# tungphambasement/TNN

Measured on AMD Instinct MI355X. Metric: images/sec (whole node) WRN-16-8 on 32x32x3, pipeline-parallel, higher is better.
Workload: dtype bf16; 1 GPU; model=cifar100_wrn16_8, global_batch=256, input=32x32x3, microbatches=1, graphed_step=True, parallelism=single

## Files before the change

tnn_amd/csrc/bindings.cpp:

```cpp

#include <array>
#include <torch/extension.h>
#include <ATen/hip/HIPContext.h>

#include "kernels.h"

namespace tnn {

static hipStream_t cur_stream() {
  return at::hip::getCurrentHIPStreamMasqueradingAsCUDA().stream();
}

static void* zero_page(const at::Tensor& like) {
  static at::Tensor z;
  if (!z.defined() || z.device() != like.device())
    z = at::zeros({16}, like.options().dtype(at::kFloat));
  return z.data_ptr();
}

static DT dt_of(const at::Tensor& t) {
  if (t.scalar_type() == at::kFloat) return DT::F32;
  if (t.scalar_type() == at::kBFloat16) return DT::BF16;
  TORCH_CHECK(false, "tnn_amd kernels support fp32/bf16, got ", t.scalar_type());
}
// ... 424 lines not shown
                                         const at::Tensor& w,
                                         const c10::optional<at::Tensor>& bias,
                                         int64_t sh, int64_t sw, int64_t ph,
                                         int64_t pw) {
  return conv2d_fwd_impl(x, w, bias, sh, sw, ph, pw, false, true);
}

at::Tensor conv2d_dgrad(const at::Tensor& dy, const at::Tensor& w, int64_t H,
                        int64_t W, int64_t sh, int64_t sw, int64_t ph,
                        int64_t pw) {
  CHECK_IN(dy);
  CHECK_IN(w);
  int KH = w.size(0), KW = w.size(1), Cin = w.size(2), Cout = w.size(3);
  auto cs = conv_shape_out(dy.size(0), H, W, Cin, Cout, KH, KW, sh, sw, ph, pw,
                           dy.size(1), dy.size(2));
  auto dx = at::empty({cs.N, H, W, Cin}, dy.options());
  if (conv2d_dgrad_wants_db(dt_of(dy), dy.data_ptr(), cs)) {
    auto w_t2d = at::empty({Cin, (int64_t)KH * KW * Cout}, w.options());
    transpose_w_dgrad_launch(dt_of(w), w.data_ptr(), w_t2d.data_ptr(), KH * KW,
                             Cin, Cout, cur_stream());
    conv2d_dgrad_launch(dt_of(dy), dy.data_ptr(), nullptr, w_t2d.data_ptr(),
                        dx.data_ptr(), zero_page(dy), cs, cur_stream());
    return dx;
  }
  auto w_t = at::empty({KH, KW, Cout, Cin}, w.options());
  transpose_w_launch(dt_of(w), w.data_ptr(), w_t.data_ptr(), KH, KW, Cin, Cout,
                     cur_stream());
  conv2d_dgrad_launch(dt_of(dy), dy.data_ptr(), w_t.data_ptr(), nullptr,
                      dx.data_ptr(), zero_page(dy), cs, cur_stream());
  return dx;
}

std::string conv2d_fwd_route_name(const at::Tensor& x, const at::Tensor& w,
                                  int64_t sh, int64_t sw, int64_t ph,
                                  int64_t pw, bool stats) {
  CHECK_IN(x);
  CHECK_IN(w);
  auto cs = conv_shape(x, w.size(2), w.size(3), w.size(0), w.size(1), sh, sw,
                       ph, pw);
  return conv2d_fwd_route(dt_of(x), x.data_ptr(), cs, stats);
}

std::string conv2d_dgrad_route_name(const at::Tensor& dy,
                                    const at::Tensor& w, int64_t H, int64_t W,
                                    int64_t sh, int64_t sw, int64_t ph,
                                    int64_t pw) {
  CHECK_IN(dy);
  CHECK_IN(w);
  auto cs = conv_shape_out(dy.size(0), H, W, w.size(2), w.size(3), w.size(0),
                           w.size(1), sh, sw, ph, pw, dy.size(1), dy.size(2));
  return conv2d_dgrad_route(dt_of(dy), dy.data_ptr(), cs);
}

static at::Tensor conv2d_wgrad_rows(const at::Tensor& x, const at::Tensor& dy,
                                    int64_t KH, int64_t KW, int64_t sh,
                                    int64_t sw, int64_t ph, int64_t pw,
                                    bool out_in_dt, bool bias) {
  CHECK_IN(x);
  CHECK_IN(dy);
  auto cs = conv_shape(x, x.size(3), dy.size(3), KH, KW, sh, sw, ph, pw);
  TORCH_CHECK(dy.size(1) == cs.OH && dy.size(2) == cs.OW, "wgrad shape");
  DT out_dt = out_in_dt ? dt_of(x) : DT::F32;
  const int64_t rows = KH * KW * cs.Cin + (bias ? 1 : 0);
  auto out = at::empty({rows, (int64_t)cs.Cout},
                       out_dt == DT::F32 ? x.options().dtype(at::kFloat)
                                         : x.options());
  int z = conv2d_wgrad_zsplits(cs);
  at::Tensor ws;
  float* wsp = nullptr;
  if (z > 1 || out_dt != DT::F32) {
    ws = at::empty({(int64_t)z * rows * cs.Cout},
                   x.options().dtype(at::kFloat));
    wsp = ws.data_ptr<float>();
  }
  conv2d_wgrad_launch(dt_of(x), x.data_ptr(), dy.data_ptr(), out.data_ptr(),
                      out_dt, wsp, z, zero_page(x), cs, bias, cur_stream());
  return out;
}

at::Tensor conv2d_wgrad(const at::Tensor& x, const at::Tensor& dy, int64_t KH,
                        int64_t KW, int64_t sh, int64_t sw, int64_t ph,
                        int64_t pw, bool out_in_dt) {
  return conv2d_wgrad_rows(x, dy, KH, KW, sh, sw, ph, pw, out_in_dt, false)
      .view({KH, KW, x.size(3), dy.size(3)});
}

std::vector<at::Tensor> conv2d_wgrad_bias(const at::Tensor& x,
                                          const at::Tensor& dy, int64_t KH,
                                          int64_t KW, int64_t sh, int64_t sw,
                                          int64_t ph, int64_t pw,
                                          bool out_in_dt) {
  auto out = conv2d_wgrad_rows(x, dy, KH, KW, sh, sw, ph, pw, out_in_dt, true);
  const int64_t kout = out.size(0) - 1;
  return {out.narrow(0, 0, kout).view({KH, KW, x.size(3), dy.size(3)}),
          out.select(0, kout)};
}

std::vector<at::Tensor> bn_fwd_train(const at::Tensor& x,
                                     const at::Tensor& gamma,
                                     const at::Tensor& beta,
                                     const c10::optional<at::Tensor>& rmean,
                                     const c10::optional<at::Tensor>& rvar,
                                     double momentum, double eps, bool relu,
                                     double dropout_p, int64_t seed,
                                     const c10::optional<at::Tensor>& precomp,
                                     const c10::optional<at::Tensor>& ctr =
                                         c10::nullopt) {
  CHECK_IN(x);
  TORCH_CHECK(dropout_p == 0.0 || relu, "fused BN dropout requires relu");
  int C = x.size(-1);
  int64_t rows = x.numel() / C;
  auto mean = at::empty({C}, x.options().dtype(at::kFloat));
  auto invstd = at::empty({C}, x.options().dtype(at::kFloat));
  auto y = at::empty_like(x);
  float* rm = rmean.has_value() ? rmean->data_ptr<float>() : nullptr;
  float* rv = rvar.has_value() ? rvar->data_ptr<float>() : nullptr;
  if (precomp.has_value()) {
    TORCH_CHECK(precomp->numel() == 2 * C, "bad precomputed stats");
    const float* ps = precomp->data_ptr<float>();
    bn_finalize_launch(ps, ps + C, mean.data_ptr<float>(),
// ... 778 lines not shown
  TORCH_CHECK(step.is_cuda() && step.scalar_type() == at::kLong &&
              step.numel() == 1, "sample_logits step must be int64 [1]");
  const float* up = nullptr;
  if (u.has_value()) {
    TORCH_CHECK(u->is_cuda() && u->is_contiguous() &&
                u->scalar_type() == at::kFloat && u->numel() == R,
                "sample_logits u must be fp32 [R] on device");
    up = u->data_ptr<float>();
  }
  auto ids = at::empty({R}, logits.options().dtype(at::kLong));
  if (R > 0)
    sample_logits_launch(logits.data_ptr(), ids.data_ptr<int64_t>(), (int)R,
                         (int)V, (float)temperature,
                         (int)std::min<int64_t>(top_k, V), (float)top_p,
                         (uint64_t)seed, step.data_ptr<int64_t>(), up,
                         cur_stream());
  return ids;
}

namespace imgcodec {
at::Tensor decode_image(const py::bytes& data);
}

}

PYBIND11_MODULE(TORCH_EXTENSION_NAME, m) {
  m.def("act_fwd", &tnn::act_fwd);
  m.def("act_bwd", &tnn::act_bwd);
  m.def("relu_bwd_mask", &tnn::relu_bwd_mask);
  m.def("add_act_fwd", &tnn::add_act_fwd);
  m.def("add_act_bwd", &tnn::add_act_bwd);
  m.def("dropout_fwd", &tnn::dropout_fwd, py::arg("x"), py::arg("p"),
        py::arg("seed"), py::arg("ctr") = c10::nullopt);
  m.def("dropout_bwd", &tnn::dropout_bwd);
  m.def("colsum", &tnn::colsum);
  m.def("gemm", &tnn::gemm, py::arg("a"), py::arg("b"), py::arg("bias"),
        py::arg("act_kind"), py::arg("residual") = c10::nullopt,
        py::arg("ln_gamma") = c10::nullopt, py::arg("ln_beta") = c10::nullopt,
        py::arg("ln_eps") = 1e-5);
  m.def("gemm_skinny", &tnn::gemm_skinny, py::arg("a"), py::arg("b"),
        py::arg("bias"), py::arg("act_kind"),
        py::arg("residual") = c10::nullopt, py::arg("ln_gamma") = c10::nullopt,
        py::arg("ln_beta") = c10::nullopt, py::arg("ln_eps") = 1e-5);
  m.def("skinny_enabled", &tnn::skinny_enabled);
  m.def("gemm_nt", &tnn::gemm_nt);
  m.def("gemm_tn", &tnn::gemm_tn);
  m.def("mfma_selftest", &tnn::mfma_selftest);
  m.def("mfma_selftest_f32", &tnn::mfma_selftest_f32);
  m.def("conv2d_fwd", &tnn::conv2d_fwd);
  m.def("conv2d_fwd_stats", &tnn::conv2d_fwd_stats);
  m.def("conv2d_dgrad", &tnn::conv2d_dgrad);
  m.def("conv2d_fwd_route", &tnn::conv2d_fwd_route_name);
  m.def("conv2d_dgrad_route", &tnn::conv2d_dgrad_route_name);
  m.def("conv2d_wgrad", &tnn::conv2d_wgrad);
  m.def("conv2d_wgrad_bias", &tnn::conv2d_wgrad_bias);
  m.def("bn_fwd_train", &tnn::bn_fwd_train, py::arg("x"), py::arg("gamma"),
        py::arg("beta"), py::arg("rmean"), py::arg("rvar"),
        py::arg("momentum"), py::arg("eps"), py::arg("relu"),
        py::arg("dropout_p"), py::arg("seed"), py::arg("precomp"),
        py::arg("ctr") = c10::nullopt);
  m.def("bn_fwd_infer", &tnn::bn_fwd_infer);
  m.def("bn_bwd", &tnn::bn_bwd, py::arg("x"), py::arg("dy"),
        py::arg("gamma"), py::arg("mean"), py::arg("invstd"),
        py::arg("y_relu"), py::arg("dy_scale"),
        py::arg("resid") = py::none());
  m.def("maxpool_fwd", &tnn::maxpool_fwd);
  m.def("maxpool_bwd", &tnn::maxpool_bwd);
  m.def("avgpool_fwd", &tnn::avgpool_fwd);
  m.def("avgpool_bwd", &tnn::avgpool_bwd);
  m.def("ce_fwd", &tnn::ce_fwd);
  m.def("ce_bwd", &tnn::ce_bwd);
  m.def("ptloss_fwd", &tnn::ptloss_fwd);
  m.def("ptloss_bwd", &tnn::ptloss_bwd);
  m.def("gn_fwd", &tnn::gn_fwd);
  m.def("gn_bwd", &tnn::gn_bwd);
  m.def("ln_fwd", &tnn::ln_fwd);
  m.def("ln_bwd", &tnn::ln_bwd, py::arg("x"), py::arg("dy"),
        py::arg("gamma"), py::arg("mean"), py::arg("invstd"),
        py::arg("resid") = py::none());
  m.def("embedding_fwd", &tnn::embedding_fwd);
  m.def("embedding_bwd", &tnn::embedding_bwd);
  m.def("attn_fwd", &tnn::attn_fwd);
  m.def("attn_bwd", &tnn::attn_bwd, py::arg("q"), py::arg("k"),
        py::arg("v"), py::arg("o"), py::arg("dout"), py::arg("lse"),
        py::arg("causal"), py::arg("dq_out") = py::none(),
        py::arg("dk_out") = py::none(), py::arg("dv_out") = py::none());
  m.def("bmm", &tnn::bmm);
  m.def("smax_fwd", &tnn::smax_fwd);
  m.def("smax_bwd", &tnn::smax_bwd);
  m.def("attn_decode", &tnn::attn_decode);
  m.def("kv_append", &tnn::kv_append);
  m.def("attn_extend", &tnn::attn_extend);
  m.def("kv_append_n", &tnn::kv_append_n);
  m.def("sample_logits", &tnn::sample_logits, py::arg("logits"),
        py::arg("temperature"), py::arg("top_k"), py::arg("top_p"),
        py::arg("seed"), py::arg("step"), py::arg("u") = c10::nullopt);
  m.def("sgd_step", &tnn::sgd_step, py::arg("param"), py::arg("master"),
        py::arg("grad"), py::arg("momentum_buf"), py::arg("lr"),
        py::arg("momentum"), py::arg("weight_decay"), py::arg("nesterov"),
        py::arg("clip") = c10::nullopt, py::arg("lr_dev") = c10::nullopt);
  m.def("adam_step", &tnn::adam_step, py::arg("param"), py::arg("master"),
        py::arg("grad"), py::arg("m"), py::arg("v"), py::arg("step"),
        py::arg("lr"), py::arg("beta1"), py::arg("beta2"), py::arg("eps"),
        py::arg("weight_decay"), py::arg("adamw"),
        py::arg("step_dev") = c10::nullopt, py::arg("clip") = c10::nullopt,
        py::arg("lr_dev") = c10::nullopt);
// ... 16 lines not shown
```

tnn_amd/csrc/conv2d.hip:

```cpp

#include "common.h"
#include "kernels.h"
#include "tile_gemm.h"

namespace tnn {

using namespace tile;

template <bool POW2>
DEV int idiv(int x, const IDiv& f) {
  if constexpr (POW2) return x >> f.lg;
  else if (f.magic)
    return (int)(((unsigned long long)(unsigned)x * f.magic) >> f.sh);
  else
    return x / f.d;
}
template <bool POW2>
DEV int imod(int x, const IDiv& f) {
  if constexpr (POW2) return x & (f.d - 1);
  else return x - idiv<POW2>(x, f) * f.d;
}

DEV void kdecode(int kidx, const ConvShape& cs, int& kh, int& kw) {
  kh = (kidx * cs.mkw16) >> 16;
// ... 167 lines not shown
  });
}

template <typename T, typename S>
DEV void conv_fwd_stats(const WaveCoordT<S>& wc, f32x4 acc[S::FM][S::FN],
                        const T* bias_p, float* stats, const ConvShape& cs,
                        int m0, int n0, int M) {
  constexpr int FM = S::FM, FN = S::FN;
  float* ssum = stats;
  float* ssumsq = stats + cs.Cout;
  const int cr = (wc.lane >> 4) * 4;
  const int cc = wc.lane & 15;
#pragma unroll
  for (int fn = 0; fn < FN; ++fn) {
    int col = n0 + wc.wcol0 + fn * 16 + cc;
    float bias = 0.0f;
    if (col < cs.Cout) {
      if (bias_p) bias = VecIO<T>::to_f32(bias_p[col]);
    }
    float s = 0.0f, ss = 0.0f;
#pragma unroll
    for (int fm = 0; fm < FM; ++fm)
#pragma unroll
      for (int j = 0; j < 4; ++j) {
        int row = m0 + wc.wrow0 + fm * 16 + cr + j;
        if (row < M && col < cs.Cout) {
          float v = acc[fm][fn][j] + bias;
          s += v;
          ss += v * v;
        }
      }
    s += __shfl_xor(s, 16, 64);
    ss += __shfl_xor(ss, 16, 64);
    s += __shfl_xor(s, 32, 64);
    ss += __shfl_xor(ss, 32, 64);
    if (wc.lane < 16 && col < cs.Cout) {
      atomicAdd(&ssum[col], s);
      atomicAdd(&ssumsq[col], ss);
    }
  }
}

template <bool POW2, typename T, bool S2, typename S>
DEV void dgrad_store(const WaveCoordT<S>& wc, f32x4 acc[S::FM][S::FN], T* DX,
                     const ConvShape& cs, const DgradClass<S2>& dc, int m0,
                     int n0) {
  epilogue_visit(wc, acc, m0, n0, [&](int row, int col, float v) {
    if (row < dc.M && col < cs.Cin)
      DX[dc.template pixel<POW2>(cs, row) * cs.Cin + col] =
          VecIO<T>::from_f32(v);
  });
}

DEV float* wgrad_slab_store(const WaveCoord& wc, f32x4 acc[FM][FN],
                            float* DW, const ConvShape& cs, int Kout,
                            int bias_row, int r0, int n0) {
  float* out = DW + (int64_t)blockIdx.z * (Kout + bias_row) * cs.Cout;
  epilogue_visit(wc, acc, r0, n0, [&](int row, int col, float v) {
    if (row < Kout && col < cs.Cout) out[(int64_t)row * cs.Cout + col] = v;
  });
  return out;
}
DEV void wgrad_colsum_store(float* out, const ConvShape& cs, int Kout, int n0,
                            float bsum) {
  bsum = colsum_tile_finish(bsum);
  int col = n0 + (threadIdx.x >> 2);
  if ((threadIdx.x & 3) == 0 && col < cs.Cout)
    out[(int64_t)Kout * cs.Cout + col] = bsum;
}

template <bool DB, typename T, typename S, typename RowFn, typename TapFn,
          typename AtFn>
DEV void conv_db_kloop(T* As0, T* As1, T* Bs0, T* Bs1,
                       const WaveCoordT<S>& wc, f32x4 acc[S::FM][S::FN],
                       const T* __restrict__ asrc, int lgSW, int lgC,
                       const T* __restrict__ bsrc, int64_t bstride,
                       int brows, int m0, int n0, int K,
                       const T* __restrict__ zero16, RowFn&& row,
                       TapFn&& tap, AtFn&& at) {
  constexpr int NA = glds_count<T, S::BM>();
  constexpr int NB = glds_count<T, S::BN>();
  constexpr int NPER = NA + NB;
  const int wid = __builtin_amdgcn_readfirstlane(wc.wid);
  const bool uni = lgC >= 6;

  const T* ab[NA];
  int ap[NA], aq[NA];
  const T* bb[NB];
  bool bok[NB];
#pragma unroll
  for (int i = 0; i < NA; ++i) {
    const int j = wid * NA + i;
    int64_t noff;
    int p, q;
    const bool ok = row(m0 + glds_row<T>(j, wc.lane), noff, p, q);
    ab[i] = asrc + noff + (uni ? glds_kk<T>(j, wc.lane) : 0);
    ap[i] = ok ? p : -(1 << 28);
    aq[i] = q;
  }
#pragma unroll
  for (int i = 0; i < NB; ++i) {
    const int j = wid * NB + i;
    const int gn = n0 + glds_row<T>(j, wc.lane);
    bok[i] = gn < brows;
    bb[i] = bsrc + (int64_t)gn * bstride + (uni ? glds_kk<T>(j, wc.lane) : 0);
  }

  auto a_ptr = [&](int i, int dh, int dw, int c, bool& ok) {
    int sh, sw;
    ok = at(ap[i], aq[i], dh, dw, sh, sw);
    const unsigned pix = ((unsigned)sh << lgSW) + (unsigned)sw;
    return ab[i] + (int)((pix << lgC) + (unsigned)c);
  };
  auto stage = [&](int t, T* a_img, T* b_img) {
// ... 451 lines not shown
      int c = threadIdx.x + it * THREADS;
      int mm = c / (BM / V);
      int rr = (c % (BM / V)) * V;
      int gm = k0 + mm, gr = r0 + rr;
      asrc[it] = gm < m_end && gr < Kout
                     ? fwd_src<true>(X, cs, fwd_row<true>(cs, gm), gr, zero16)
                     : zero16;
    }
    const T* bsrc[RB];
#pragma unroll
    for (int it = 0; it < RB; ++it) {
      int c = threadIdx.x + it * THREADS;
      int mm = c / (BN / V);
      int nn = (c % (BN / V)) * V;
      int gm = k0 + mm;
      bsrc[it] = (gm < m_end && n0 + nn + V <= cs.Cout)
                     ? &DY[(int64_t)gm * cs.Cout + n0 + nn]
                     : zero16;
    }
#pragma unroll
    for (int it = 0; it < RA; ++it) va[it] = *(const VecT*)asrc[it];
#pragma unroll
    for (int it = 0; it < RB; ++it) vb[it] = *(const VecT*)bsrc[it];
  };

  load_tile(m_begin);
  for (int k0 = m_begin; k0 < m_end; k0 += BK) {
#pragma unroll
    for (int it = 0; it < RA; ++it) {
      int c = threadIdx.x + it * THREADS;
      int mm = c / (BM / V);
      int rr = (c % (BM / V)) * V;
#pragma unroll
      for (int j = 0; j < V; ++j) As[lds_off<T>(rr + j, mm)] = va[it].e[j];
    }
#pragma unroll
    for (int it = 0; it < RB; ++it) {
      int c = threadIdx.x + it * THREADS;
      int mm = c / (BN / V);
      int nn = (c % (BN / V)) * V;
#pragma unroll
      for (int j = 0; j < V; ++j) Bs[lds_off<T>(nn + j, mm)] = vb[it].e[j];
    }
    if (k0 + BK < m_end) load_tile(k0 + BK);
    __syncthreads();
    mfma_compute_tile(As, Bs, wc, acc);
    if (colsum) bsum += colsum_tile_partial(Bs);
    __syncthreads();
  }
  float* out = wgrad_slab_store(wc, acc, DW, cs, Kout, bias_row, r0, n0);
  if (colsum) wgrad_colsum_store(out, cs, Kout, n0, bsum);
}

__launch_bounds__(THREADS, 2)
__global__ void k_conv_wgrad_tr(const bf16* __restrict__ X,
                                const bf16* __restrict__ DY,
                                float* __restrict__ DW,
                                const bf16* __restrict__ zero16, ConvShape cs,
                                int bias_row) {
  constexpr int NA = glds_kmajor_count<BM / 8>();
  constexpr int NPER = NA + glds_kmajor_count<BN / 8>();
  __shared__ alignas(16) bf16 As0[BK * BM], As1[BK * BM];
  __shared__ alignas(16) bf16 Bs0[BK * BN], Bs1[BK * BN];
  const int M = cs.N * cs.OH * cs.OW;
  const int Kout = cs.KH * cs.KW * cs.Cin;
  int tr_, tn_;
  conv_tile_order(cs, tr_, tn_);
  const int r0 = tr_ * BM;
  const int n0 = tn_ * BN;
  const int m_begin = (int)((int64_t)M * blockIdx.z / gridDim.z);
  const int m_end = (int)((int64_t)M * (blockIdx.z + 1) / gridDim.z);
  const WaveCoord wc;
  const int wm = wc.wid / WAVES_N;
  f32x4 acc[FM][FN] = {};
  const bool colsum = bias_row && tr_ == 0;
  f32x4 bacc = {};
  bf16x8 ones;
#pragma unroll
  for (int j = 0; j < 8; ++j) ones[j] = (__bf16)1.0f;

  int a_dh[NA], a_dw[NA], a_ci[NA];
#pragma unroll
  for (int i = 0; i < NA; ++i) {
    const int row = 4 * (wc.wid * NA + i) + wc.lane / 16;
    const int gr = r0 + 8 * ((wc.lane % 16) ^ kmaj_key<16>(row));
    int kh, kw;
    kdecode(gr >> cs.d_cin.lg, cs, kh, kw);
    a_dh[i] = kh - cs.PH;
    a_dw[i] = kw - cs.PW;
    a_ci[i] = gr < Kout ? (gr & (cs.Cin - 1)) : -1;
  }

  auto stage = [&](int k0, bf16* a_img, bf16* b_img) {
    glds_stage_kmajor<BM / 8>(a_img, wc,
                              [&](int i, int row, int) -> const bf16* {
      const int gm = k0 + row;
      const int n = gm >> cs.d_ohow.lg;
      const int rem = gm & (cs.OH * cs.OW - 1);
      const int oh = rem >> cs.d_ow.lg, ow = rem & (cs.OW - 1);
      const int ih = oh * cs.SH + a_dh[i];
      const int iw = ow * cs.SW + a_dw[i];
      const bool ok = gm < m_end && a_ci[i] >= 0 &&
                      (unsigned)ih < (unsigned)cs.H &&
                      (unsigned)iw < (unsigned)cs.W;
      const int pix = (n << cs.d_hw.lg) + (ih << cs.d_w.lg) + iw;
      const bf16* p = X + (((int64_t)pix << cs.d_cin.lg) + a_ci[i]);
      return ok ? p : zero16;
    });
    glds_stage_kmajor<BN / 8>(b_img, wc,
                              [&](int, int row, int ch) -> const bf16* {
      const int gm = k0 + row, gn = n0 + 8 * ch;
      const bf16* p = DY + (((int64_t)gm << cs.d_cout.lg) + gn);
      return gm < m_end && gn < cs.Cout ? p : zero16;
    });
  };
  auto compute = [&](const bf16* a_img, const bf16* b_img) {
#pragma unroll
    for (int ks = 0; ks < BK / 32; ++ks) {
      TrFrag a[FM], b[FN];
#pragma unroll
      for (int fm = 0; fm < FM; ++fm)
        a[fm] = tr_frag_issue<BM / 8>(a_img, ks * 32, wc.wrow0 + fm * 16,
                                      wc.lane);
#pragma unroll
      for (int fn = 0; fn < FN; ++fn)
        b[fn] = tr_frag_issue<BN / 8>(b_img, ks * 32, wc.wcol0 + fn * 16,
                                      wc.lane);
      tr_frags_wait(a, b);
#pragma unroll
      for (int fm = 0; fm < FM; ++fm)
#pragma unroll
        for (int fn = 0; fn < FN; ++fn)
          acc[fm][fn] = __builtin_amdgcn_mfma_f32_16x16x32_bf16(
              a[fm].get(), b[fn].get(), acc[fm][fn], 0, 0, 0);
      if (colsum)
        bacc = __builtin_amdgcn_mfma_f32_16x16x32_bf16(
            ones, wm ? b[1].get() : b[0].get(), bacc, 0, 0, 0);
    }
  };

  auto step = [&](int k0, bf16* a_cur, bf16* b_cur, bf16* a_nxt,
                  bf16* b_nxt) {
    if (k0 + BK < m_end) {
      stage(k0 + BK, a_nxt, b_nxt);
      wait_vmcnt<NPER>();
    } else {
      wait_vmcnt<0>();
    }
    __builtin_amdgcn_s_barrier();
    compute(a_cur, b_cur);
    __builtin_amdgcn_s_barrier();
  };
  if (m_begin < m_end) stage(m_begin, As0, Bs0);
  for (int k0 = m_begin; k0 < m_end; k0 += 2 * BK) {
    step(k0, As0, Bs0, As1, Bs1);
    if (k0 + BK < m_end) step(k0 + BK, As1, Bs1, As0, Bs0);
  }

  float* out = wgrad_slab_store(wc, acc, DW, cs, Kout, bias_row, r0, n0);
  if (colsum && wc.lane < 16) {
    int col = n0 + wc.wcol0 + 16 * wm + wc.lane;
    if (col < cs.Cout) out[(int64_t)Kout * cs.Cout + col] = bacc[0];
  }
}

template <typename T>
__global__ void k_transpose2d_tiled(const T* __restrict__ in,
                                    T* __restrict__ out, int rows, int cols) {
  __shared__ T tile[32][33];
  const int c0 = blockIdx.x * 32, r0 = blockIdx.y * 32;
  const int64_t slice = (int64_t)blockIdx.z * rows * cols;
  const T* src = in + slice;
  T* dst = out + slice;
  const int tx = threadIdx.x & 31, ty = threadIdx.x >> 5;
#pragma unroll
  for (int d = 0; d < 32; d += 8) {
    int r = r0 + ty + d, c = c0 + tx;
    if (r < rows && c < cols) tile[ty + d][tx] = src[(int64_t)r * cols + c];
  }
  __syncthreads();
#pragma unroll
  for (int d = 0; d < 32; d += 8) {
    int c = c0 + ty + d, r = r0 + tx;
    if (c < cols && r < rows) dst[(int64_t)c * rows + r] = tile[tx][ty + d];
  }
}

template <typename T>
__global__ void k_transpose_w_dgrad(const T* __restrict__ W,
                                    T* __restrict__ WT2D, int KHW, int Cin,
                                    int Cout) {
  int64_t i = (int64_t)blockIdx.x * blockDim.x + threadIdx.x;
  int64_t n = (int64_t)KHW * Cin * Cout;
  if (i >= n) return;
  int co = i % Cout;
  int ci = (i / Cout) % Cin;
  int64_t khw = i / ((int64_t)Cin * Cout);
  WT2D[((int64_t)ci * KHW + khw) * Cout + co] = W[i];
}

template <typename T>
__global__ void k_transpose_w_dgrad_vec(const T* __restrict__ W,
                                        T* __restrict__ WT2D, int KHW,
                                        int Cin, int Cout) {
  constexpr int V = 16 / sizeof(T);
  struct alignas(16) P { T e[16 / sizeof(T)]; };
  const int cov = Cout / V;
  int64_t i = (int64_t)blockIdx.x * blockDim.x + threadIdx.x;
  int64_t n = (int64_t)KHW * Cin * cov;
  if (i >= n) return;
  int c = i % cov;
  int ci = (i / cov) % Cin;
  int64_t khw = i / ((int64_t)Cin * cov);
  ((P*)WT2D)[((int64_t)ci * KHW + khw) * cov + c] =
      ((const P*)W)[((int64_t)khw * Cin + ci) * cov + c];
// ... 223 lines not shown
  dim3 grid(ceil_div(M, BM), ceil_div(cs.Cin, BN));
  bool p2 = all_pow2(cs);
  bool g = p2 && vec_ok(dt, dy, cs.Cout);
  bool s1 = cs.SH == 1 && cs.SW == 1;
  ConvShape cs2;
  bool s2 = dgrad_parity(cs, cs2);
  int Mc = cs.N * (cs.H / 2) * (cs.W / 2);
  dim3 grid_s2(ceil_div(Mc, BM), ceil_div(cs.Cin, BN), 4);
  const Wide wide = dgrad_wide(dt, w_t2d != nullptr, s2, cs);
  dispatch_dt(dt, [&](auto tag) {
    using T = typename decltype(tag)::type;
    auto DY = (const T*)dy;
    auto DX = (T*)dx;
    auto Z = (const T*)zero16;
    if constexpr (sizeof(T) == 2) {
      if (wide != Wide::NO) {
        auto WT = (const T*)w_t2d;
        constexpr int WBM = TileWide::BM, WBN = TileWide::BN;
        const bool sb = wide == Wide::SB;
        if (s2)
          return launch(sb ? k_conv_dgrad_sb_wide<true>
                           : k_conv_dgrad_db_wide<true>,
                        dim3(ceil_div(Mc, WBM), cs.Cin / WBN, 4), s, DY, WT,
                        DX, Z, cs2);
        dim3 gw(ceil_div(M, WBM), cs.Cin / WBN);
        if (s1)
          return launch(sb ? k_conv_dgrad_sb_wide<false, true>
                           : k_conv_dgrad_db_wide<false, true>,
                        gw, s, DY, WT, DX, Z, cs);
        return launch(sb ? k_conv_dgrad_sb_wide<> : k_conv_dgrad_db_wide<>,
                      gw, s, DY, WT, DX, Z, cs);
      }
    }
    if (w_t2d) {
      auto WT = (const T*)w_t2d;
      if (s2)
        return launch(k_conv_dgrad_db<T, true>, grid_s2, s, DY, WT, DX, Z,
                      cs2);
      return launch(s1 ? k_conv_dgrad_db<T, false, true> : k_conv_dgrad_db<T>,
                    grid, s, DY, WT, DX, Z, cs);
    }
    auto WT = (const T*)w_t;
    if (g && s2)
      return launch(k_conv_dgrad<T, true, true, true>, grid_s2, s, DY, WT, DX,
                    Z, cs2);
    launch(g ? (s1 ? k_conv_dgrad<T, true, true, false, true>
                   : k_conv_dgrad<T, true, true>)
             : (p2 ? k_conv_dgrad<T, true, false>
                   : k_conv_dgrad<T, false, false>),
           grid, s, DY, WT, DX, Z, cs);
  });
}

int conv2d_wgrad_zsplits(const ConvShape& cs) {
  int M = cs.N * cs.OH * cs.OW;
  int Kout = cs.KH * cs.KW * cs.Cin;
  int base = ceil_div(Kout, BM) * ceil_div(cs.Cout, BN);
  int want = 2048;
  int z = base >= want ? 1
                       : std::min(ceil_div(M, 4 * BK), ceil_div(want, base));
  return std::max(z, 1);
}

void conv2d_wgrad_launch(DT dt, const void* x, const void* dy, void* dw_out,
                         DT out_dt, float* ws, int z, const void* zero16,
                         const ConvShape& cs, bool bias, hipStream_t s) {
  int Kout = cs.KH * cs.KW * cs.Cin;
  const int bias_row = bias ? 1 : 0;
  bool direct = z == 1 && out_dt == DT::F32;
  float* target = direct ? (float*)dw_out : ws;
  dim3 grid(ceil_div(Kout, BM), ceil_div(cs.Cout, BN), z);
  bool p2 = all_pow2(cs);
  bool vec = p2 && vec_ok(dt, x, cs.Cin) && vec_ok(dt, dy, cs.Cout);
  dispatch_dt(dt, [&](auto tag) {
    using T = typename decltype(tag)::type;
    auto X = (const T*)x;
    auto DY = (const T*)dy;
    auto Z = (const T*)zero16;
    if (vec) {
      if constexpr (sizeof(T) == 2)
        launch(k_conv_wgrad_tr, grid, s, X, DY, target, Z, cs, bias_row);
      else
        launch(k_conv_wgrad_vec<T>, grid, s, X, DY, target, Z, cs, bias_row);
      return;
    }
    launch(p2 ? k_conv_wgrad<T, true> : k_conv_wgrad<T, false>, grid, s, X,
           DY, target, cs, bias_row);
  });
  if (!direct)
    splitk_reduce_launch(ws, dw_out, out_dt, z,
                         (int64_t)(Kout + bias_row) * cs.Cout, s,
                         (int64_t)Kout * cs.Cout);
}

}
```

tnn_amd/csrc/kernels.h:

```cpp
#pragma once

#include <hip/hip_runtime.h>
#ifdef __HIPCC__
#include <hip/hip_bf16.h>
#endif
#include <algorithm>
#include <cstdint>

namespace tnn {

enum class DT { F32, BF16 };

inline bool ptr_aligned16(const void* p) { return ((uintptr_t)p & 15) == 0; }

inline int vec_elems(DT dt) { return dt == DT::F32 ? 4 : 8; }

#ifdef __HIPCC__
template <typename T> struct TypeTag { using type = T; };
template <typename F>
inline void dispatch_dt(DT dt, F&& f) {
  if (dt == DT::F32) f(TypeTag<float>{});
  else f(TypeTag<__hip_bfloat16>{});
}
#endif
// ... 62 lines not shown
                          int64_t n, hipStream_t s, int64_t n_shape = 0);
void mfma_selftest_launch(const void* a_bf16, const void* b_bf16, float* d,
                          hipStream_t s);
void mfma_selftest_f32_launch(const float* a, const float* b, float* d,
                              hipStream_t s);

struct IDiv {
  int d = 1;
  int lg = 0;
  int sh = 0;
  unsigned long long magic = 0;
  void set(int dd) {
    d = dd;
    lg = (dd & (dd - 1)) == 0 ? __builtin_ctz(dd) : -1;
    magic = 0;
    sh = 0;
    if (lg < 0 && dd > 1 && dd < 65536) {
      sh = dd < 1024 ? 36 : 42;
      magic = ((1ull << sh) + dd - 1) / dd;
    }
  }
};

struct ConvShape {
  int N, H, W, Cin, Cout, KH, KW, SH, SW, PH, PW, OH, OW;
  IDiv d_ohow, d_ow, d_cin, d_hw, d_w, d_cout;
  int mkw16;
  void init_fdiv() {
    d_ohow.set(OH * OW);
    d_ow.set(OW);
    d_cin.set(Cin);
    d_hw.set(H * W);
    d_w.set(W);
    d_cout.set(Cout);
    mkw16 = 65536 / KW + 1;
  }
};
bool conv2d_fwd_wants_db(DT dt, const void* x, const ConvShape& cs);
void transpose_w_fwd_launch(DT dt, const void* w, void* w_t2, int KHW, int Cin,
                            int Cout, hipStream_t s);
void conv2d_fwd_launch(DT dt, const void* x, const void* w, const void* w_t2,
                       const void* bias, void* y, const void* zero16,
                       float* stats, const ConvShape& cs, bool relu,
                       hipStream_t s);
bool conv2d_dgrad_wants_db(DT dt, const void* dy, const ConvShape& cs);
const char* conv2d_fwd_route(DT dt, const void* x, const ConvShape& cs,
                             bool stats);
const char* conv2d_dgrad_route(DT dt, const void* dy, const ConvShape& cs);
void transpose_w_dgrad_launch(DT dt, const void* w, void* w_t2d, int KHW,
                              int Cin, int Cout, hipStream_t s);
void conv2d_dgrad_launch(DT dt, const void* dy, const void* w_t,
                         const void* w_t2d, void* dx, const void* zero16,
                         const ConvShape& cs, hipStream_t s);
int conv2d_wgrad_zsplits(const ConvShape& cs);
void conv2d_wgrad_launch(DT dt, const void* x, const void* dy, void* dw_out,
                         DT out_dt, float* ws, int z, const void* zero16,
                         const ConvShape& cs, bool bias, hipStream_t s);
void transpose_w_launch(DT dt, const void* w, void* w_t, int KH, int KW,
                        int Cin, int Cout, hipStream_t s);

int64_t bn_stats_ws_floats(DT dt, const void* x, int64_t rows, int cols);
void bn_stats_launch(DT dt, const void* x, float* mean, float* invstd,
                     float* rmean, float* rvar, float momentum, float* ws,
                     int64_t rows, int cols, float eps, hipStream_t s);
void bn_finalize_launch(const float* sum, const float* sumsq, float* mean,
                        float* invstd, float* rmean, float* rvar,
                        float momentum, int64_t rows, int cols, float eps,
                        hipStream_t s);
void bn_apply_launch(DT dt, const void* x, const float* mean,
                     const float* invstd, const float* gamma, const float* beta,
                     void* y, int64_t rows, int cols, bool relu, hipStream_t s);
void bn_apply_drop_launch(DT dt, const void* x, const float* mean,
                          const float* invstd, const float* gamma,
                          const float* beta, void* y, int64_t rows, int cols,
                          float p, uint64_t seed, const int64_t* ctr,
                          hipStream_t s);
void bn_infer_launch(DT dt, const void* x, const float* rmean,
                     const float* rvar, const float* gamma, const float* beta,
                     void* y, int64_t rows, int cols, float eps, bool relu,
                     hipStream_t s);
int64_t bn_bwd_ws_floats(DT dt, const void* x, const void* dy, int64_t rows,
                         int cols);
void bn_bwd_reduce_launch(DT dt, const void* x, const void* dy, const void* y_relu,
                          const float* mean, const float* invstd, float* sum_dy,
                          float* sum_dy_xhat, float* ws, int64_t rows, int cols,
                          float dy_scale, hipStream_t s);
void bn_bwd_apply_launch(DT dt, const void* x, const void* dy, const void* y_relu,
                         const float* mean, const float* invstd,
                         const float* gamma, const float* sum_dy,
                         const float* sum_dy_xhat, void* dx, const void* resid,
                         int64_t rows, int cols, float dy_scale,
                         hipStream_t s);

struct PoolShape {
  int N, H, W, C, KH, KW, SH, SW, PH, PW, OH, OW;
};
void maxpool_fwd_launch(DT dt, const void* x, void* y, int32_t* idx,
                        const PoolShape& ps, hipStream_t s);
void maxpool_bwd_launch(DT dt, const void* dy, const int32_t* idx, float* dx_f32,
                        const PoolShape& ps, hipStream_t s);
void avgpool_fwd_launch(DT dt, const void* x, void* y, const PoolShape& ps,
                        hipStream_t s);
void avgpool_bwd_launch(DT dt, const void* dy, void* dx, const PoolShape& ps,
                        hipStream_t s);

void ce_fwd_launch(DT dt, const void* logits, const int64_t* targets,
                   float* loss, float* lse, int64_t rows, int cols,
// ... 109 lines not shown
```

tnn_amd/csrc/tile_gemm.h:

```cpp
#pragma once

#include "common.h"

namespace tile {

constexpr int BK = 64, THREADS = 256;

template <int BM_, int BN_, int WAVES_M_ = 2, int WAVES_N_ = 2>
struct TileShape {
  static constexpr int BM = BM_, BN = BN_;
  static constexpr int WAVES_M = WAVES_M_, WAVES_N = WAVES_N_;
  static constexpr int WM = BM / WAVES_M;
  static constexpr int WN = BN / WAVES_N;
  static constexpr int FM = WM / 16;
  static constexpr int FN = WN / 16;
  static_assert(WAVES_M * WAVES_N * 64 == THREADS, "one wave per sub-tile");
  static_assert(WM % 16 == 0 && WN % 16 == 0, "whole 16x16 fragments");
};
using TileStd = TileShape<128, 64>;
using TileWide = TileShape<128, 128>;

constexpr int BM = TileStd::BM, BN = TileStd::BN;
constexpr int WAVES_M = TileStd::WAVES_M, WAVES_N = TileStd::WAVES_N;
constexpr int WM = TileStd::WM;
// ... 211 lines not shown
  for (int ks = 0; ks < BK / 32; ++ks) {
    RmFrag a[FM], b[FN];
#pragma unroll
    for (int fm = 0; fm < FM; ++fm)
      a[fm] = rm_frag_issue(As, w.wrow0 + fm * 16, ks * 32, w.lane);
#pragma unroll
    for (int fn = 0; fn < FN; ++fn)
      b[fn] = rm_frag_issue(Bs, w.wcol0 + fn * 16, ks * 32, w.lane);
    rm_frags_wait(a, b);
#pragma unroll
    for (int fm = 0; fm < FM; ++fm)
#pragma unroll
      for (int fn = 0; fn < FN; ++fn)
        acc[fm][fn] = __builtin_amdgcn_mfma_f32_16x16x32_bf16(
            a[fm].get(), b[fn].get(), acc[fm][fn], 0, 0, 0);
  }
}

template <typename T>
DEV int glds_row(int j, int lane) {
  constexpr int ROWB = BK * (int)sizeof(T);
  return (1024 / ROWB) * j + lane / (ROWB / 16);
}
template <typename T>
DEV int glds_kk(int j, int lane) {
  constexpr int LPR = BK * (int)sizeof(T) / 16;
  const int rl = glds_row<T>(j, lane);
  const int byte = ((lane % LPR) * 16) ^ ((((rl >> 3) ^ rl) & 7) << 4);
  return byte / (int)sizeof(T);
}
template <typename T>
DEV void glds_issue(T* img, int j, const T* src) {
  __builtin_amdgcn_global_load_lds(
      (const __attribute__((address_space(1))) unsigned int*)src,
      (__attribute__((address_space(3))) unsigned int*)
          &img[j * (1024 / (int)sizeof(T))],
      16, 0, 0);
}

using s16x4 = __attribute__((ext_vector_type(4))) short;

template <int NCH>
DEV int kmaj_key(int row) {
  static_assert(NCH == 16 || NCH == 8, "128- or 64-column bf16 image");
  if constexpr (NCH == 16) return ((row & 3) << 2) | ((row >> 2) & 3);
  else return (row & 2) | (((row >> 3) & 1) << 2);
}

template <int NCH>
DEV int kmaj_off(int row, int ch) {
  return 16 * NCH * row + 16 * (ch ^ kmaj_key<NCH>(row));
}

template <int NCH, typename AddrFn>
DEV void glds_stage_kmajor(bf16* img, const WaveCoord& w, AddrFn&& addr) {
  constexpr int RPK = 64 / NCH;
  constexpr int NPW = BK * NCH * 16 / 1024 / 4;
#pragma unroll
  for (int i = 0; i < NPW; ++i) {
    const int j = __builtin_amdgcn_readfirstlane(w.wid) * NPW + i;
    const int row = RPK * j + w.lane / NCH;
    const int ch = (w.lane % NCH) ^ kmaj_key<NCH>(row);
    const bf16* src = addr(i, row, ch);
    __builtin_amdgcn_global_load_lds(
        (const __attribute__((address_space(1))) unsigned int*)src,
        (__attribute__((address_space(3))) unsigned int*)&img[j * 512], 16, 0,
        0);
  }
}
template <int NCH>
constexpr int glds_kmajor_count() { return BK * NCH * 16 / 1024 / 4; }

struct TrFrag {
  s16x4 lo, hi;
  DEV bf16x8 get() const {
    s16x8 v = __builtin_shufflevector(lo, hi, 0, 1, 2, 3, 4, 5, 6, 7);
    return __builtin_bit_cast(bf16x8, v);
  }
};

template <int NCH>
DEV TrFrag tr_frag_issue(const bf16* img, int krow0, int col0, int lane) {
  typedef __attribute__((address_space(3))) const char* lds_p;
  const int g = lane >> 4, q = (lane >> 2) & 3, p = lane & 3;
  const int row = krow0 + 16 * (g >> 1) + 8 * (g & 1) + q;
  const int ch = (col0 >> 3) + (p >> 1);
  const unsigned base = (unsigned)(size_t)(lds_p)(const char*)img + 8 * (p & 1);
  TrFrag f;
  asm volatile("ds_read_b64_tr_b16 %0, %1"
               : "=v"(f.lo) : "v"(base + kmaj_off<NCH>(row, ch)) : "memory");
  asm volatile("ds_read_b64_tr_b16 %0, %1"
               : "=v"(f.hi) : "v"(base + kmaj_off<NCH>(row + 4, ch)) : "memory");
  return f;
}

DEV void tr_frags_wait(TrFrag (&a)[FM], TrFrag (&b)[FN]) {
  static_assert(FM == 4 && FN == 2, "operand list below");
  asm volatile("s_waitcnt lgkmcnt(0)"
               : "+v"(a[0].lo), "+v"(a[0].hi), "+v"(a[1].lo), "+v"(a[1].hi),
                 "+v"(a[2].lo), "+v"(a[2].hi), "+v"(a[3].lo), "+v"(a[3].hi),
                 "+v"(b[0].lo), "+v"(b[0].hi), "+v"(b[1].lo), "+v"(b[1].hi)
               :: "memory");
}

static_assert(THREADS == 4 * BN, "4 threads per B-tile column");
template <typename T>
DEV float colsum_tile_partial(const T* Bs) {
  constexpr int V = 16 / (int)sizeof(T);
  const int co = threadIdx.x >> 2;
  const int m0 = (threadIdx.x & 3) * (BK / 4);
  float s = 0.0f;
#pragma unroll
  for (int c = 0; c < BK / 4; c += V) {
    Pack16<T> v = *(const Pack16<T>*)&Bs[lds_off<T>(co, m0 + c)];
#pragma unroll
    for (int j = 0; j < V; ++j) s += VecIO<T>::to_f32(v.e[j]);
  }
  return s;
}

DEV float colsum_tile_finish(float s) {
  s += __shfl_xor(s, 1, 64);
  s += __shfl_xor(s, 2, 64);
  return s;
}

template <typename S, typename F>
DEV void epilogue_visit(const WaveCoordT<S>& w, f32x4 acc[S::FM][S::FN],
                        int row0, int col0, F&& emit) {
  constexpr int FM = S::FM, FN = S::FN;
  const int cr = (w.lane >> 4) * 4;
  const int cc = w.lane & 15;
#pragma unroll
  for (int fm = 0; fm < FM; ++fm)
#pragma unroll
    for (int fn = 0; fn < FN; ++fn)
#pragma unroll
      for (int j = 0; j < 4; ++j) {
        int row = row0 + w.wrow0 + fm * 16 + cr + j;
        int col = col0 + w.wcol0 + fn * 16 + cc;
        emit(row, col, acc[fm][fn][j]);
      }
}

}
```

Measured before the change: 43330 img/s.

## Add wide 128x128 bf16 wgrad tile with single/double-buffer routing and split tuning

Adds a 128x128-tile variant of the transposed-LDS bf16 weight-gradient kernel, in single- and double-buffered forms, and routes eligible convolutions to it using a heuristic based on tile count and split capacity. The wider tile is meant to raise MFMA operand reuse per LDS load and cut the number of blocks. Split-K counts for the wide route are now set from occupancy slot budgets. The single-buffered variant gives up load/compute overlap in exchange for lower LDS use and higher occupancy. Env knobs and a route-name binding are added for inspection and tuning.

```diff
diff --git a/tnn_amd/csrc/bindings.cpp b/tnn_amd/csrc/bindings.cpp
--- a/tnn_amd/csrc/bindings.cpp
+++ b/tnn_amd/csrc/bindings.cpp
@@ -500,6 +500,16 @@
   return conv2d_dgrad_route(dt_of(dy), dy.data_ptr(), cs);
 }
 
+std::tuple<std::string, int64_t> conv2d_wgrad_route_name(
+    const at::Tensor& x, const at::Tensor& dy, int64_t KH, int64_t KW,
+    int64_t sh, int64_t sw, int64_t ph, int64_t pw) {
+  CHECK_IN(x);
+  CHECK_IN(dy);
+  auto cs = conv_shape(x, x.size(3), dy.size(3), KH, KW, sh, sw, ph, pw);
+  return {conv2d_wgrad_route(dt_of(x), x.data_ptr(), dy.data_ptr(), cs),
+          conv2d_wgrad_zsplits(dt_of(x), x.data_ptr(), dy.data_ptr(), cs)};
+}
+
 static at::Tensor conv2d_wgrad_rows(const at::Tensor& x, const at::Tensor& dy,
                                     int64_t KH, int64_t KW, int64_t sh,
                                     int64_t sw, int64_t ph, int64_t pw,
@@ -513,7 +523,7 @@
   auto out = at::empty({rows, (int64_t)cs.Cout},
                        out_dt == DT::F32 ? x.options().dtype(at::kFloat)
                                          : x.options());
-  int z = conv2d_wgrad_zsplits(cs);
+  int z = conv2d_wgrad_zsplits(dt_of(x), x.data_ptr(), dy.data_ptr(), cs);
   at::Tensor ws;
   float* wsp = nullptr;
   if (z > 1 || out_dt != DT::F32) {
@@ -1398,6 +1408,7 @@
   m.def("conv2d_dgrad", &tnn::conv2d_dgrad);
   m.def("conv2d_fwd_route", &tnn::conv2d_fwd_route_name);
   m.def("conv2d_dgrad_route", &tnn::conv2d_dgrad_route_name);
+  m.def("conv2d_wgrad_route", &tnn::conv2d_wgrad_route_name);
   m.def("conv2d_wgrad", &tnn::conv2d_wgrad);
   m.def("conv2d_wgrad_bias", &tnn::conv2d_wgrad_bias);
   m.def("bn_fwd_train", &tnn::bn_fwd_train, py::arg("x"), py::arg("gamma"),
diff --git a/tnn_amd/csrc/conv2d.hip b/tnn_amd/csrc/conv2d.hip
--- a/tnn_amd/csrc/conv2d.hip
+++ b/tnn_amd/csrc/conv2d.hip
@@ -243,14 +243,30 @@
   });
 }
 
-DEV float* wgrad_slab_store(const WaveCoord& wc, f32x4 acc[FM][FN],
-                            float* DW, const ConvShape& cs, int Kout,
-                            int bias_row, int r0, int n0) {
+template <typename S>
+DEV float* wgrad_slab_store(const WaveCoordT<S>& wc,
+                            f32x4 acc[S::FM][S::FN], float* DW,
+                            const ConvShape& cs, int Kout, int bias_row,
+                            int r0, int n0) {
   float* out = DW + (int64_t)blockIdx.z * (Kout + bias_row) * cs.Cout;
   epilogue_visit(wc, acc, r0, n0, [&](int row, int col, float v) {
     if (row < Kout && col < cs.Cout) out[(int64_t)row * cs.Cout + col] = v;
   });
   return out;
+}
+template <typename S>
+DEV void wgrad_biasrow_store(float* out, const WaveCoordT<S>& wc,
+                             const f32x4 (&bacc)[S::FN / S::WAVES_M],
+                             const ConvShape& cs, int Kout, int n0) {
+  constexpr int NBF = S::FN / S::WAVES_M;
+  const int wm = wc.wid / S::WAVES_N;
+  if (wc.lane < 16) {
+#pragma unroll
+    for (int t = 0; t < NBF; ++t) {
+      int col = n0 + wc.wcol0 + 16 * (NBF * wm + t) + wc.lane;
+      if (col < cs.Cout) out[(int64_t)Kout * cs.Cout + col] = bacc[t][0];
+    }
+  }
 }
 DEV void wgrad_colsum_store(float* out, const ConvShape& cs, int Kout, int n0,
                             float bsum) {
@@ -808,29 +824,33 @@
   if (colsum) wgrad_colsum_store(out, cs, Kout, n0, bsum);
 }
 
-__launch_bounds__(THREADS, 2)
-__global__ void k_conv_wgrad_tr(const bf16* __restrict__ X,
-                                const bf16* __restrict__ DY,
-                                float* __restrict__ DW,
-                                const bf16* __restrict__ zero16, ConvShape cs,
-                                int bias_row) {
-  constexpr int NA = glds_kmajor_count<BM / 8>();
-  constexpr int NPER = NA + glds_kmajor_count<BN / 8>();
-  __shared__ alignas(16) bf16 As0[BK * BM], As1[BK * BM];
-  __shared__ alignas(16) bf16 Bs0[BK * BN], Bs1[BK * BN];
+template <bool DB, typename S>
+DEV void conv_wgrad_tr_tile(bf16* As0, bf16* As1, bf16* Bs0, bf16* Bs1,
+                            const bf16* __restrict__ X,
+                            const bf16* __restrict__ DY,
+                            float* __restrict__ DW,
+                            const bf16* __restrict__ zero16,
+                            const ConvShape& cs, int bias_row) {
+  constexpr int FM = S::FM, FN = S::FN;
+  constexpr int ACH = S::BM / 8, BCH = S::BN / 8;
+  static_assert(ACH == 16, "the hoisted A decode below is for 128-row tiles");
+  static_assert(S::WAVES_M == 2, "bias row: wm selects half the fragments");
+  constexpr int NA = glds_kmajor_count<ACH>();
+  constexpr int NPER = NA + glds_kmajor_count<BCH>();
+  constexpr int NBF = FN / S::WAVES_M;
   const int M = cs.N * cs.OH * cs.OW;
   const int Kout = cs.KH * cs.KW * cs.Cin;
   int tr_, tn_;
   conv_tile_order(cs, tr_, tn_);
-  const int r0 = tr_ * BM;
-  const int n0 = tn_ * BN;
+  const int r0 = tr_ * S::BM;
+  const int n0 = tn_ * S::BN;
   const int m_begin = (int)((int64_t)M * blockIdx.z / gridDim.z);
   const int m_end = (int)((int64_t)M * (blockIdx.z + 1) / gridDim.z);
-  const WaveCoord wc;
-  const int wm = wc.wid / WAVES_N;
+  const WaveCoordT<S> wc;
+  const int wm = wc.wid / S::WAVES_N;
   f32x4 acc[FM][FN] = {};
   const bool colsum = bias_row && tr_ == 0;
-  f32x4 bacc = {};
+  f32x4 bacc[NBF] = {};
   bf16x8 ones;
 #pragma unroll
   for (int j = 0; j < 8; ++j) ones[j] = (__bf16)1.0f;
@@ -848,8 +868,8 @@
   }
 
   auto stage = [&](int k0, bf16* a_img, bf16* b_img) {
-    glds_stage_kmajor<BM / 8>(a_img, wc,
-                              [&](int i, int row, int) -> const bf16* {
+    glds_stage_kmajor<ACH>(a_img, wc,
+                           [&](int i, int row, int) -> const bf16* {
       const int gm = k0 + row;
       const int n = gm >> cs.d_ohow.lg;
       const int rem = gm & (cs.OH * cs.OW - 1);
@@ -863,8 +883,8 @@
       const bf16* p = X + (((int64_t)pix << cs.d_cin.lg) + a_ci[i]);
       return ok ? p : zero16;
     });
-    glds_stage_kmajor<BN / 8>(b_img, wc,
-                              [&](int, int row, int ch) -> const bf16* {
+    glds_stage_kmajor<BCH>(b_img, wc,
+                           [&](int, int row, int ch) -> const bf16* {
       const int gm = k0 + row, gn = n0 + 8 * ch;
       const bf16* p = DY + (((int64_t)gm << cs.d_cout.lg) + gn);
       return gm < m_end && gn < cs.Cout ? p : zero16;
@@ -876,22 +896,25 @@
       TrFrag a[FM], b[FN];
 #pragma unroll
       for (int fm = 0; fm < FM; ++fm)
-        a[fm] = tr_frag_issue<BM / 8>(a_img, ks * 32, wc.wrow0 + fm * 16,
-                                      wc.lane);
+        a[fm] = tr_frag_issue<ACH>(a_img, ks * 32, wc.wrow0 + fm * 16,
+                                   wc.lane);
 #pragma unroll
       for (int fn = 0; fn < FN; ++fn)
-        b[fn] = tr_frag_issue<BN / 8>(b_img, ks * 32, wc.wcol0 + fn * 16,
-                                      wc.lane);
-      tr_frags_wait(a, b);
+        b[fn] = tr_frag_issue<BCH>(b_img, ks * 32, wc.wcol0 + fn * 16,
+                                   wc.lane);
+      tr_frags_wait<S>(a, b);
 #pragma unroll
       for (int fm = 0; fm < FM; ++fm)
 #pragma unroll
         for (int fn = 0; fn < FN; ++fn)
           acc[fm][fn] = __builtin_amdgcn_mfma_f32_16x16x32_bf16(
               a[fm].get(), b[fn].get(), acc[fm][fn], 0, 0, 0);
-      if (colsum)
-        bacc = __builtin_amdgcn_mfma_f32_16x16x32_bf16(
-            ones, wm ? b[1].get() : b[0].get(), bacc, 0, 0, 0);
+      if (colsum) {
+#pragma unroll
+        for (int t = 0; t < NBF; ++t)
+          bacc[t] = __builtin_amdgcn_mfma_f32_16x16x32_bf16(
+              ones, wm ? b[NBF + t].get() : b[t].get(), bacc[t], 0, 0, 0);
+      }
     }
   };
 
@@ -907,16 +930,55 @@
     compute(a_cur, b_cur);
     __builtin_amdgcn_s_barrier();
   };
-  if (m_begin < m_end) stage(m_begin, As0, Bs0);
-  for (int k0 = m_begin; k0 < m_end; k0 += 2 * BK) {
-    step(k0, As0, Bs0, As1, Bs1);
-    if (k0 + BK < m_end) step(k0 + BK, As1, Bs1, As0, Bs0);
+  if constexpr (DB) {
+    if (m_begin < m_end) stage(m_begin, As0, Bs0);
+    for (int k0 = m_begin; k0 < m_end; k0 += 2 * BK) {
+      step(k0, As0, Bs0, As1, Bs1);
+      if (k0 + BK < m_end) step(k0 + BK, As1, Bs1, As0, Bs0);
+    }
+  } else {
+    for (int k0 = m_begin; k0 < m_end; k0 += BK) {
+      stage(k0, As0, Bs0);
+      wait_vmcnt<0>();
+      __builtin_amdgcn_s_barrier();
+      compute(As0, Bs0);
+      __builtin_amdgcn_s_barrier();
+    }
   }
 
   float* out = wgrad_slab_store(wc, acc, DW, cs, Kout, bias_row, r0, n0);
-  if (colsum && wc.lane < 16) {
-    int col = n0 + wc.wcol0 + 16 * wm + wc.lane;
-    if (col < cs.Cout) out[(int64_t)Kout * cs.Cout + col] = bacc[0];
+  if (colsum) wgrad_biasrow_store<S>(out, wc, bacc, cs, Kout, n0);
+}
+
+__launch_bounds__(THREADS, 2)
+__global__ void k_conv_wgrad_tr(const bf16* __restrict__ X,
+                                const bf16* __restrict__ DY,
+                                float* __restrict__ DW,
+                                const bf16* __restrict__ zero16, ConvShape cs,
+                                int bias_row) {
+  __shared__ alignas(16) bf16 As0[BK * BM], As1[BK * BM];
+  __shared__ alignas(16) bf16 Bs0[BK * BN], Bs1[BK * BN];
+  conv_wgrad_tr_tile<true, TileStd>(As0, As1, Bs0, Bs1, X, DY, DW, zero16, cs,
+                                    bias_row);
+}
+
+template <bool DB>
+__launch_bounds__(THREADS, DB ? 2 : 3)
+__global__ void k_conv_wgrad_tr_wide(const bf16* __restrict__ X,
+                                     const bf16* __restrict__ DY,
+                                     float* __restrict__ DW,
+                                     const bf16* __restrict__ zero16,
+                                     ConvShape cs, int bias_row) {
+  constexpr int WBM = TileWide::BM, WBN = TileWide::BN;
+  if constexpr (DB) {
+    __shared__ alignas(16) bf16 As0[BK * WBM], As1[BK * WBM];
+    __shared__ alignas(16) bf16 Bs0[BK * WBN], Bs1[BK * WBN];
+    conv_wgrad_tr_tile<true, TileWide>(As0, As1, Bs0, Bs1, X, DY, DW, zero16,
+                                       cs, bias_row);
+  } else {
+    __shared__ alignas(16) bf16 As0[BK * WBM], Bs0[BK * WBN];
+    conv_wgrad_tr_tile<false, TileWide>(As0, As0, Bs0, Bs0, X, DY, DW, zero16,
+                                        cs, bias_row);
   }
 }
 
@@ -1246,14 +1308,92 @@
   });
 }
 
-int conv2d_wgrad_zsplits(const ConvShape& cs) {
-  int M = cs.N * cs.OH * cs.OW;
-  int Kout = cs.KH * cs.KW * cs.Cin;
+static int wgrad_wide_mode() {
+  static const int mode = env_int("TNN_WGRAD_WIDE", 1);
+  return mode;
+}
+static int wgrad_wide_buf() {
+  static const int buf = env_int("TNN_WGRAD_WIDE_BUF", 0);
+  return buf;
+}
+static int wgrad_splits_pin() {
+  static const int z = env_int("TNN_WGRAD_SPLITS", 0);
+  return z;
+}
+
+enum class WgradRoute { TR_WIDE_DB, TR_WIDE_SB, TR, VEC, POW2, GENERIC };
+
+constexpr int WGRAD_WIDE_WAVES = 1;
+constexpr int WGRAD_WIDE_1TILE_MAXKOUT = 144;
+constexpr int WGRAD_WIDE_SB_MINTILES = 144;
+constexpr int WGRAD_WIDE_DB_SLOTS = 512, WGRAD_WIDE_SB_SLOTS = 768;
+static int wgrad_wide_waves() {
+  static const int n =
+      std::max(env_int("TNN_WGRAD_WAVES", WGRAD_WIDE_WAVES), 1);
+  return n;
+}
+static Wide wgrad_wide_auto(const ConvShape& cs) {
+  const int Kout = cs.KH * cs.KW * cs.Cin;
+  const int nt = cs.Cout / TileWide::BN;
+  const int tiles = ceil_div(Kout, TileWide::BM) * nt;
+  const int cap = ceil_div(cs.N * cs.OH * cs.OW, 4 * BK);
+  if (nt == 1 && Kout > WGRAD_WIDE_1TILE_MAXKOUT) return Wide::NO;
+  if (cap < WGRAD_WIDE_DB_SLOTS / tiles) return Wide::NO;
+  return tiles >= WGRAD_WIDE_SB_MINTILES ? Wide::SB : Wide::DB;
+}
+static Wide wgrad_wide(const ConvShape& cs) {
+  if (cs.Cout % TileWide::BN != 0 || wgrad_wide_mode() == 0) return Wide::NO;
+  Wide pick = wgrad_wide_auto(cs);
+  if (wgrad_wide_mode() == 1 && pick == Wide::NO) return Wide::NO;
+  if (wgrad_wide_buf() != 0)
+    pick = wgrad_wide_buf() == 2 ? Wide::SB : Wide::DB;
+  else if (pick == Wide::NO)
+    pick = Wide::DB;
+  return pick;
+}
+
+static WgradRoute wgrad_route(DT dt, const void* x, const void* dy,
+                              const ConvShape& cs) {
+  const bool p2 = all_pow2(cs);
+  if (p2 && vec_ok(dt, x, cs.Cin) && vec_ok(dt, dy, cs.Cout)) {
+    if (dt != DT::BF16) return WgradRoute::VEC;
+    const Wide wide = wgrad_wide(cs);
+    if (wide == Wide::NO) return WgradRoute::TR;
+    return wide == Wide::SB ? WgradRoute::TR_WIDE_SB : WgradRoute::TR_WIDE_DB;
+  }
+  return p2 ? WgradRoute::POW2 : WgradRoute::GENERIC;
+}
+
+int conv2d_wgrad_zsplits(DT dt, const void* x, const void* dy,
+                         const ConvShape& cs) {
+  const int M = cs.N * cs.OH * cs.OW;
+  const int Kout = cs.KH * cs.KW * cs.Cin;
+  const int cap = std::max(ceil_div(M, 4 * BK), 1);
+  if (wgrad_splits_pin() > 0) return std::min(wgrad_splits_pin(), cap);
+  const WgradRoute route = wgrad_route(dt, x, dy, cs);
+  if (route == WgradRoute::TR_WIDE_DB || route == WgradRoute::TR_WIDE_SB) {
+    const int base = ceil_div(Kout, TileWide::BM) * (cs.Cout / TileWide::BN);
+    const int slots = (route == WgradRoute::TR_WIDE_DB ? WGRAD_WIDE_DB_SLOTS
+                                                       : WGRAD_WIDE_SB_SLOTS) *
+                      wgrad_wide_waves();
+    return std::max(std::min(cap, slots / base), 1);
+  }
   int base = ceil_div(Kout, BM) * ceil_div(cs.Cout, BN);
   int want = 2048;
-  int z = base >= want ? 1
-                       : std::min(ceil_div(M, 4 * BK), ceil_div(want, base));
+  int z = base >= want ? 1 : std::min(cap, ceil_div(want, base));
   return std::max(z, 1);
+}
+
+const char* conv2d_wgrad_route(DT dt, const void* x, const void* dy,
+                               const ConvShape& cs) {
+  switch (wgrad_route(dt, x, dy, cs)) {
+    case WgradRoute::TR_WIDE_DB: return "k_conv_wgrad_tr_wide<db>";
+    case WgradRoute::TR_WIDE_SB: return "k_conv_wgrad_tr_wide<sb>";
+    case WgradRoute::TR: return "k_conv_wgrad_tr";
+    case WgradRoute::VEC: return "k_conv_wgrad_vec";
+    case WgradRoute::POW2: return "k_conv_wgrad<pow2>";
+    default: return "k_conv_wgrad";
+  }
 }
 
 void conv2d_wgrad_launch(DT dt, const void* x, const void* dy, void* dw_out,
@@ -1264,22 +1404,31 @@
   bool direct = z == 1 && out_dt == DT::F32;
   float* target = direct ? (float*)dw_out : ws;
   dim3 grid(ceil_div(Kout, BM), ceil_div(cs.Cout, BN), z);
-  bool p2 = all_pow2(cs);
-  bool vec = p2 && vec_ok(dt, x, cs.Cin) && vec_ok(dt, dy, cs.Cout);
+  const WgradRoute route = wgrad_route(dt, x, dy, cs);
   dispatch_dt(dt, [&](auto tag) {
     using T = typename decltype(tag)::type;
     auto X = (const T*)x;
     auto DY = (const T*)dy;
     auto Z = (const T*)zero16;
-    if (vec) {
-      if constexpr (sizeof(T) == 2)
-        launch(k_conv_wgrad_tr, grid, s, X, DY, target, Z, cs, bias_row);
-      else
-        launch(k_conv_wgrad_vec<T>, grid, s, X, DY, target, Z, cs, bias_row);
-      return;
-    }
-    launch(p2 ? k_conv_wgrad<T, true> : k_conv_wgrad<T, false>, grid, s, X,
-           DY, target, cs, bias_row);
+    if constexpr (sizeof(T) == 2) {
+      if (route == WgradRoute::TR_WIDE_DB || route == WgradRoute::TR_WIDE_SB)
+        return launch(route == WgradRoute::TR_WIDE_DB
+                          ? k_conv_wgrad_tr_wide<true>
+                          : k_conv_wgrad_tr_wide<false>,
+                      dim3(ceil_div(Kout, TileWide::BM),
+                           cs.Cout / TileWide::BN, z),
+                      s, X, DY, target, Z, cs, bias_row);
+      if (route == WgradRoute::TR)
+        return launch(k_conv_wgrad_tr, grid, s, X, DY, target, Z, cs,
+                      bias_row);
+    } else {
+      if (route == WgradRoute::VEC)
+        return launch(k_conv_wgrad_vec<T>, grid, s, X, DY, target, Z, cs,
+                      bias_row);
+    }
+    launch(route == WgradRoute::POW2 ? k_conv_wgrad<T, true>
+                                     : k_conv_wgrad<T, false>,
+           grid, s, X, DY, target, cs, bias_row);
   });
   if (!direct)
     splitk_reduce_launch(ws, dw_out, out_dt, z,
diff --git a/tnn_amd/csrc/kernels.h b/tnn_amd/csrc/kernels.h
--- a/tnn_amd/csrc/kernels.h
+++ b/tnn_amd/csrc/kernels.h
@@ -138,7 +138,10 @@
 void conv2d_dgrad_launch(DT dt, const void* dy, const void* w_t,
                          const void* w_t2d, void* dx, const void* zero16,
                          const ConvShape& cs, hipStream_t s);
-int conv2d_wgrad_zsplits(const ConvShape& cs);
+const char* conv2d_wgrad_route(DT dt, const void* x, const void* dy,
+                               const ConvShape& cs);
+int conv2d_wgrad_zsplits(DT dt, const void* x, const void* dy,
+                         const ConvShape& cs);
 void conv2d_wgrad_launch(DT dt, const void* x, const void* dy, void* dw_out,
                          DT out_dt, float* ws, int z, const void* zero16,
                          const ConvShape& cs, bool bias, hipStream_t s);
diff --git a/tnn_amd/csrc/tile_gemm.h b/tnn_amd/csrc/tile_gemm.h
--- a/tnn_amd/csrc/tile_gemm.h
+++ b/tnn_amd/csrc/tile_gemm.h
@@ -287,8 +287,8 @@
   return 16 * NCH * row + 16 * (ch ^ kmaj_key<NCH>(row));
 }
 
-template <int NCH, typename AddrFn>
-DEV void glds_stage_kmajor(bf16* img, const WaveCoord& w, AddrFn&& addr) {
+template <int NCH, typename S = TileStd, typename AddrFn>
+DEV void glds_stage_kmajor(bf16* img, const WaveCoordT<S>& w, AddrFn&& addr) {
   constexpr int RPK = 64 / NCH;
   constexpr int NPW = BK * NCH * 16 / 1024 / 4;
 #pragma unroll
@@ -329,13 +329,23 @@
   return f;
 }
 
-DEV void tr_frags_wait(TrFrag (&a)[FM], TrFrag (&b)[FN]) {
-  static_assert(FM == 4 && FN == 2, "operand list below");
-  asm volatile("s_waitcnt lgkmcnt(0)"
-               : "+v"(a[0].lo), "+v"(a[0].hi), "+v"(a[1].lo), "+v"(a[1].hi),
-                 "+v"(a[2].lo), "+v"(a[2].hi), "+v"(a[3].lo), "+v"(a[3].hi),
-                 "+v"(b[0].lo), "+v"(b[0].hi), "+v"(b[1].lo), "+v"(b[1].hi)
-               :: "memory");
+template <typename S = TileStd>
+DEV void tr_frags_wait(TrFrag (&a)[S::FM], TrFrag (&b)[S::FN]) {
+  static_assert(S::FM == 4 && (S::FN == 2 || S::FN == 4),
+                "operand lists below");
+  if constexpr (S::FN == 2)
+    asm volatile("s_waitcnt lgkmcnt(0)"
+                 : "+v"(a[0].lo), "+v"(a[0].hi), "+v"(a[1].lo), "+v"(a[1].hi),
+                   "+v"(a[2].lo), "+v"(a[2].hi), "+v"(a[3].lo), "+v"(a[3].hi),
+                   "+v"(b[0].lo), "+v"(b[0].hi), "+v"(b[1].lo), "+v"(b[1].hi)
+                 :: "memory");
+  else
+    asm volatile("s_waitcnt lgkmcnt(0)"
+                 : "+v"(a[0].lo), "+v"(a[0].hi), "+v"(a[1].lo), "+v"(a[1].hi),
+                   "+v"(a[2].lo), "+v"(a[2].hi), "+v"(a[3].lo), "+v"(a[3].hi),
+                   "+v"(b[0].lo), "+v"(b[0].hi), "+v"(b[1].lo), "+v"(b[1].hi),
+                   "+v"(b[2].lo), "+v"(b[2].hi), "+v"(b[3].lo), "+v"(b[3].hi)
+                 :: "memory");
 }
 
 static_assert(THREADS == 4 * BN, "4 threads per B-tile column");
```

Measured after the change: 44970 img/s, median of 6. +3.8%, better.
